# musbenlahrech/reporter

Measured on AMD Instinct MI355X. Metric: GPS points map-matched/sec (node) at 1/2/4/8 MI355X; % of HBM peak, higher is better.
Workload: dtype f32 geometry / f64 Viterbi + times / u64 (dist,time) route keys

## Files before the change

reporter_amd/csrc/engine.hip:

```cpp
#include <hip/hip_runtime.h>
#include <hipcub/hipcub.hpp>

#include <algorithm>
#include <chrono>
#include <cstdlib>
#include <cstring>
#include <functional>
#include <thread>
#include <type_traits>

#include "engine.hpp"
#include "json_points.hpp"

namespace rm {

const char* const kKernelNames[kNumKernels] = {"states", "candidates", "scan", "routes",
                                               "viterbi", "paths", "segments", "report", "locality",
                                               "points"};

namespace {

constexpr uint32_t kEmpty = 0xffffffffu;
constexpr int kWave = 64;
constexpr int kBigH = 4096;
// ... 196 lines not shown
  if (k == 0 && lane < kCtlWords) b.ctl[lane] = 0u;
  const uint32_t o = b.trace_off[k], n = b.trace_off[k + 1] - o;
  const MatchOptions op = b.opts[b.trace_opt[k]];
  const double interp = (double)op.interpolation_distance;
  uint32_t ns = 0, last = 0;
  float llon = 0.f, llat = 0.f;
  double lsin = 0.0, lcos = 0.0;
  float c1lo = 0.f, c1la = 0.f, c2lo = 0.f, c2la = 0.f;
  const uint32_t nl = n ? n - 1u : 0u;
  float nlo = b.lon[o + min((uint32_t)lane, nl)], nla = b.lat[o + min((uint32_t)lane, nl)];
  double ntm = b.time[o + min((uint32_t)lane, nl)];
  bool w_slot = false, w_state = false, w_gc = false;
  uint32_t w_i = 0, w_si = 0;
  double w_gcv = 0.0, w_tm = 0.0;
  for (uint32_t c0 = 0; c0 < n; c0 += 64) {
    const uint32_t i = c0 + lane, m = min(64u, n - c0);
    const bool act = i < n;
    float lo = act ? nlo : 0.f, la = act ? nla : 0.f;
    double tm = act ? ntm : 0.0;
    __asm__ volatile("" : "+v"(lo), "+v"(la), "+v"(tm) : : "memory");
    if (w_slot) { b.slot_trace[o + w_i] = k; b.choice[o + w_i] = -1; b.path_cnt[o + w_i] = 0u; }
    if (w_state) { b.state_orig[o + w_si] = w_i; b.state_time[o + w_si] = w_tm; }
    if (w_gc) b.gc[o + w_si] = w_gcv;
    __asm__ volatile("" : : : "memory");
    nlo = b.lon[o + min(i + 64u, nl)];
    nla = b.lat[o + min(i + 64u, nl)];
    ntm = b.time[o + min(i + 64u, nl)];
    w_slot = act;
    w_i = i;
    float lo1 = __shfl_up(lo, 1, 64), la1 = __shfl_up(la, 1, 64);
    float lo2 = __shfl_up(lo, 2, 64), la2 = __shfl_up(la, 2, 64);
    if (lane == 0) { lo1 = c1lo; la1 = c1la; lo2 = c2lo; la2 = c2la; }
    if (lane == 1) { lo2 = c1lo; la2 = c1la; }
    const double s0 = lat_sin(la), k0 = lat_cos(la);
    double s1 = __shfl_up(s0, 1, 64), k1 = __shfl_up(k0, 1, 64), s2 = __shfl_up(s0, 2, 64), k2 = __shfl_up(k0, 2, 64);
    if (lane <= 1) {
      const float cl = lane == 0 ? c2la : c1la;
      s2 = lat_sin(cl); k2 = lat_cos(cl);
      if (lane == 0) { s1 = lat_sin(c1la); k1 = lat_cos(c1la); }
    }
    const double d1 = gc_trig(lo1, la1, s1, k1, lo, la, s0, k0);
    const double d2 = gc_trig(lo2, la2, s2, k2, lo, la, s0, k0);
    const bool a1 = act && (i == 0 || !(d1 < interp));
    const bool a2 = act && i >= 2 && !(d2 < interp);
    const unsigned long long A = __ballot(a1), B = __ballot(a2);
    unsigned long long st = 0;
    const uint32_t last0 = last;
    double dx = 0.0;
    for (uint32_t q = 0; q < m;) {
      const uint32_t ii = c0 + q;
      if (ii == 0 || last + 1 == ii) {
        const unsigned long long rest = ~(A >> q);
        const uint32_t run = min(rest ? (uint32_t)__builtin_ctzll(rest) : 64u, m - q);
        if (run) {
          st |= (run == 64u ? ~0ull : ((1ull << run) - 1ull)) << q;
          q += run;
          last = c0 + q - 1;
        } else {
          ++q;
        }
        continue;
      }
      if (last + 2 == ii) {
        if ((B >> q) & 1ull) { st |= 1ull << q; last = ii; }
        ++q;
        continue;
      }
      float plo = llon, pla = llat;
      double ps = lsin, pc = lcos;
      if (last >= c0) {
        plo = lane_f(lo, last - c0); pla = lane_f(la, last - c0);
        ps = lane_d(s0, last - c0); pc = lane_d(k0, last - c0);
      }
      const double dv = gc_trig(plo, pla, ps, pc, lo, la, s0, k0);
      const unsigned long long far = __ballot(act && !(dv < interp)) & (~0ull << q);
      if (!far) { q = m; break; }
      const uint32_t nq = (uint32_t)__builtin_ctzll(far);
      st |= 1ull << nq;
      last = c0 + nq;
      if (lane == (int)nq) dx = dv;
      q = nq + 1;
    }
    w_state = ((st >> lane) & 1ull) != 0ull;
    w_tm = tm;
    w_gc = false;
    if (w_state) {
      const unsigned long long below = st & ((1ull << lane) - 1ull);
      const uint32_t si = ns + (uint32_t)__popcll(below);
      w_si = si;
      if (si > 0) {
        const uint32_t prev = below ? c0 + 63u - (uint32_t)__builtin_clzll(below) : last0;
        w_gc = true;
        w_gcv = i - prev == 1u ? d1 : (i - prev == 2u ? d2 : dx);
      }
    }
    ns += (uint32_t)__popcll(st);
    if (last >= c0) {
      llon = lane_f(lo, last - c0); llat = lane_f(la, last - c0);
      lsin = lane_d(s0, last - c0); lcos = lane_d(k0, last - c0);
    }
    c1lo = lane_f(lo, 63); c1la = lane_f(la, 63);
    c2lo = lane_f(lo, 62); c2la = lane_f(la, 62);
  }
  if (w_slot) { b.slot_trace[o + w_i] = k; b.choice[o + w_i] = -1; b.path_cnt[o + w_i] = 0u; }
  if (w_state) { b.state_orig[o + w_si] = w_i; b.state_time[o + w_si] = w_tm; }
  if (w_gc) b.gc[o + w_si] = w_gcv;
  if (lane == 0) b.n_states[k] = ns;
}

struct CandSmem {
  uint32_t road[kCandH];
  unsigned long long best[kCandH];
  uint32_t cell_lo[64], cell_hi[64];
  uint32_t used, ovf, ncell, slot_n;
  uint32_t list[kCandH];
};

__device__ __forceinline__ void project_rel(float ax, float ay, uint32_t acum, float bx, float by, uint32_t bcum,
                                            float& sq, uint32_t& s) {
  const float dx = bx - ax, dy = by - ay;
  const float l2 = dx * dx + dy * dy;
  float t = 0.0f;
  if (l2 > 0.0f) {
    t = -(ax * dx + ay * dy) / l2;
    if (t < 0.0f) t = 0.0f;
    if (t > 1.0f) t = 1.0f;
  }
  const float cx = ax + t * dx, cy = ay + t * dy;
  sq = cx * cx + cy * cy;
  const float along = (float)acum + t * (float)(bcum - acum);
  uint32_t v = (uint32_t)rintf(along);
  if (v < acum) v = acum;
  if (v > bcum) v = bcum;
  s = v;
}
__device__ __forceinline__ void project(float alon, float alat, uint32_t acum, float blon, float blat, uint32_t bcum,
                                        float lon, float lat, float mlon, float mlat, float& sq, uint32_t& s) {
  project_rel((alon - lon) * mlon, (alat - lat) * mlat, acum, (blon - lon) * mlon, (blat - lat) * mlat, bcum, sq, s);
}
#ifndef RM_K1_REJECT
#define RM_K1_REJECT 0
#endif
__device__ __forceinline__ bool outside_pad(float ax, float ay, float bx, float by, float pad) {
  if (!RM_K1_REJECT) return false;
  return (ax > pad && bx > pad) || (ax < -pad && bx < -pad) || (ay > pad && by > pad) || (ay < -pad && by < -pad);
}

__device__ __forceinline__ uint32_t time_ms_dev(uint32_t d_cm, uint32_t dkph) {
  if (d_cm > 11930464u) return time_ms(d_cm, dkph);
  const uint32_t D = dkph ? dkph : 1u;
  return (uint32_t)((double)(d_cm * 360u) / (double)D);
}

__device__ __forceinline__ void desc_from_rec(const uint4& a, const uint4& c, uint32_t road, uint32_t s, int mode,
                                              uint32_t acc, uint4& d0, uint4& d1) {
  uint32_t spf = (a.w != kNone && edge_ok(c.y, acc)) ? mode_speed_dkph(mode, c.y & 0xffffu) : 0u;
  uint32_t spr = (c.x != kNone && edge_ok(c.z, acc)) ? mode_speed_dkph(mode, c.z & 0xffffu) : 0u;
  if (a.w != kNone && edge_ok(c.y, acc) && spf == 0u) spf = 1u;
  if (c.x != kNone && edge_ok(c.z, acc) && spr == 0u) spr = 1u;
  d0 = make_uint4(road, s, a.z, spf | (spr << 16));
  d1 = make_uint4(a.x, a.y, spf ? time_ms_dev(s, spf) : 0xffffffffu, spr ? time_ms_dev(a.z - s, spr) : 0xffffffffu);
}

__device__ __forceinline__ void make_desc(const DevGraph& g, uint32_t road, uint32_t s, int mode, uint4& d0,
                                          uint4& d1) {
  desc_from_rec(g.road_rec[2 * (uint64_t)road], g.road_rec[2 * (uint64_t)road + 1], road, s, mode, mode_access(mode),
                d0, d1);
}

__device__ __forceinline__ void put_cand(const DevGraph& g, const DevBatch& b, uint64_t p, uint32_t rank, uint32_t road,
                                         uint32_t s, float sq, int mode) {
  uint4 d0, d1;
  make_desc(g, road, s, mode, d0, d1);
  const uint64_t at = p * kMaxCand + rank;
  b.cand_desc[2 * at] = d0;
  b.cand_desc[2 * at + 1] = d1;
  b.cand_sq[at] = sq;
}

#define K1_UNIFORM_STOP(c) (__ballot(c) == 0ull)

#ifndef RM_K1_ROWS
#define RM_K1_ROWS 4
#endif
constexpr int kK1Rows = RM_K1_ROWS;
#ifndef RM_K1_BATCH
#define RM_K1_BATCH 4
#endif
constexpr int kK1Batch = RM_K1_BATCH;
#ifndef RM_K1_SLOTS
#define RM_K1_SLOTS 16
#endif
constexpr int kK1Slots = RM_K1_SLOTS;
static_assert(kK1Slots % 4 == 0 && kK1Slots <= kMaxCand, "K1 slots");
#ifndef RM_K1_WPE
#define RM_K1_WPE 1
#endif
__global__ void __launch_bounds__(256) __attribute__((amdgpu_waves_per_eu(RM_K1_WPE))) k_candidates_lane(DevGraph g, DevBatch b) {
  uint64_t p = (uint64_t)blockIdx.x * blockDim.x + threadIdx.x;
  if (b.perm) {
    const uint64_t r = (uint64_t)xcd_block(blockIdx.x, gridDim.x) * blockDim.x + threadIdx.x;
    if (r >= b.P) return;
    p = b.perm[r];
  }
  if (p >= b.P) return;
  const uint32_t k = b.slot_trace[p];
  const uint32_t o = b.trace_off[k];
  const uint32_t s = (uint32_t)(p - o);
  if (s >= b.n_states[k]) return;
  const MatchOptions op = b.opts[b.trace_opt[k]];
  const uint32_t acc = mode_access(op.mode);
  const uint32_t pt = o + b.state_orig[p];
  const float lon = b.lon[pt], lat = b.lat[pt];
  const float r = point_radius(op, b.acc[pt]);
  const float mlon = meters_per_lon(lat);
  const float mlat = (float)kMetersPerDegLat;
  const float r2 = r * r;
  const float pad = r * 1.01f + 0.5f;
  const float qlon = pad / mlon, qlat = pad / mlat;
  const double fx0 = floor(((double)(lon - qlon) - g.lon0) / g.dlon);
  const double fx1 = floor(((double)(lon + qlon) - g.lon0) / g.dlon);
  const double fy0 = floor(((double)(lat - qlat) - g.lat0) / g.dlat);
  const double fy1 = floor(((double)(lat + qlat) - g.lat0) / g.dlat);
  uint32_t rroad[kK1Slots], rs[kK1Slots];
  unsigned long long rbest[kK1Slots];
  uint32_t n = 0;
  bool ovf = false;
  if (!(fx1 < 0 || fy1 < 0 || fx0 > (double)(g.ncx - 1) || fy0 > (double)(g.ncy - 1))) {
    const uint32_t x0 = fx0 < 0 ? 0u : (uint32_t)fx0, y0 = fy0 < 0 ? 0u : (uint32_t)fy0;
    const uint32_t x1 = fx1 > (double)(g.ncx - 1) ? g.ncx - 1 : (uint32_t)fx1;
    const uint32_t y1 = fy1 > (double)(g.ncy - 1) ? g.ncy - 1 : (uint32_t)fy1;
    for (uint32_t w0 = y0; w0 <= y1 && !ovf; w0 += kK1Rows) {
      const uint32_t nrow = min(y1 - w0 + 1u, (uint32_t)kK1Rows);
      uint32_t ra[kK1Rows], re[kK1Rows], base[kK1Rows], end[kK1Rows];
#pragma unroll
      for (int r = 0; r < kK1Rows; ++r) {
        const uint32_t cy = w0 + min((uint32_t)r, nrow - 1u);
        ra[r] = g.cell_off[cy * g.ncx + x0];
        re[r] = g.cell_off[cy * g.ncx + x1 + 1];
      }
      uint32_t tot = 0;
#pragma unroll
      for (int r = 0; r < kK1Rows; ++r) {
        base[r] = ra[r] - tot;
        tot += (uint32_t)r < nrow ? re[r] - ra[r] : 0u;
        end[r] = tot;
      }
      for (uint32_t q0 = 0; q0 < tot && !ovf; q0 += kK1Batch) {
        uint4 r0[kK1Batch], r1[kK1Batch];
#pragma unroll
        for (int y = 0; y < kK1Batch; ++y) {
          const uint32_t q = min(q0 + (uint32_t)y, tot - 1u);
          uint32_t bq = base[0];
#pragma unroll
          for (int r = 1; r < kK1Rows; ++r)
            if (q >= end[r - 1]) bq = base[r];
          const uint64_t it = bq + q;
          r0[y] = g.cell_rec[2 * it];
          r1[y] = g.cell_rec[2 * it + 1];
        }
#pragma unroll
        for (int y = 0; y < kK1Batch; ++y) {
          if (q0 + y >= tot || ovf) break;
          if (!((r1[y].z >> 29) & acc)) continue;
          const float ax = (as_f(r0[y].x) - lon) * mlon, ay = (as_f(r0[y].y) - lat) * mlat;
          const float bx = (as_f(r0[y].z) - lon) * mlon, by = (as_f(r0[y].w) - lat) * mlat;
          if (outside_pad(ax, ay, bx, by, pad)) continue;
          float sq; uint32_t sc;
          project_rel(ax, ay, r1[y].x, bx, by, r1[y].y, sq, sc);
          if (!(sq <= r2)) continue;
          const uint32_t road = r1[y].z & 0x1fffffffu;
          const unsigned long long key = ((unsigned long long)__float_as_uint(sq) << 32) | r1[y].w;
          bool found = false;
#pragma unroll
          for (int x = 0; x < kK1Slots; ++x) {
            if (K1_UNIFORM_STOP(x < (int)n)) break;
            if (x < (int)n && rroad[x] == road) {
              found = true;
              if (key < rbest[x]) { rbest[x] = key; rs[x] = sc; }
            }
          }
          if (found) continue;
          if (n >= (uint32_t)kK1Slots) { ovf = true; break; }
#pragma unroll
          for (int x = 0; x < kK1Slots; ++x) {
            if (K1_UNIFORM_STOP(x <= (int)n)) break;
            if (x == (int)n) { rroad[x] = road; rbest[x] = key; rs[x] = sc; }
          }
          ++n;
        }
      }
    }
  }
  if (ovf) {
    const uint32_t q = atomicAdd(&b.ctl[kCtlK1LaneToWave], 1u);
    b.rl_cand[q] = (uint32_t)p;
    return;
  }
  const uint32_t cacc = mode_access(op.mode);
#pragma unroll
  for (int x0 = 0; x0 < kK1Slots; x0 += 4) {
    if (K1_UNIFORM_STOP(x0 < (int)n)) break;
    if (x0 >= (int)n) break;
    uint4 ra[4], rc[4];
#pragma unroll
    for (int y = 0; y < 4; ++y) {
      const uint64_t road = rroad[min(x0 + y, (int)n - 1)];
      ra[y] = g.road_rec[2 * road];
      rc[y] = g.road_rec[2 * road + 1];
    }
#pragma unroll
    for (int y = 0; y < 4; ++y) {
      const int x = x0 + y;
      if (x >= (int)n) break;
      const uint32_t sqb = (uint32_t)(rbest[x] >> 32);
      const unsigned long long kx = ((unsigned long long)sqb << 32) | rroad[x];
      uint32_t rank = 0;
#pragma unroll
      for (int z = 0; z < kK1Slots; ++z) {
        if (K1_UNIFORM_STOP(z < (int)n)) break;
        if (z >= (int)n) continue;
        rank += ((((rbest[z] >> 32) << 32) | rroad[z]) < kx) ? 1u : 0u;
      }
      uint4 d0, d1;
      desc_from_rec(ra[y], rc[y], rroad[x], rs[x], op.mode, cacc, d0, d1);
      const uint64_t at = p * kMaxCand + rank;
      b.cand_desc[2 * at] = d0;
      b.cand_desc[2 * at + 1] = d1;
      b.cand_sq[at] = __uint_as_float(sqb);
    }
  }
  b.cand_n[p] = (uint8_t)n;
}

__device__ void cand_wave_one(const DevGraph& g, const DevBatch& b, CandSmem& sm, uint64_t p) {
  const int lane = threadIdx.x;
  const uint32_t k = b.slot_trace[p];
  const uint32_t o = b.trace_off[k];
  const MatchOptions op = b.opts[b.trace_opt[k]];
  const uint32_t acc = mode_access(op.mode);
  const uint32_t pt = o + b.state_orig[p];
  const float lon = b.lon[pt], lat = b.lat[pt];
  const float r = point_radius(op, b.acc[pt]);
  const float mlon = meters_per_lon(lat);
  const float mlat = (float)kMetersPerDegLat;
  const float r2 = r * r;
  const float pad = r * 1.01f + 0.5f;
  const float qlon = pad / mlon, qlat = pad / mlat;
  const double fx0 = floor(((double)(lon - qlon) - g.lon0) / g.dlon);
  const double fx1 = floor(((double)(lon + qlon) - g.lon0) / g.dlon);
  const double fy0 = floor(((double)(lat - qlat) - g.lat0) / g.dlat);
  const double fy1 = floor(((double)(lat + qlat) - g.lat0) / g.dlat);
  for (int h = lane; h < kCandH; h += kWave) { sm.road[h] = kEmpty; sm.best[h] = ~0ull; }
  if (lane == 0) { sm.used = 0; sm.ovf = 0; }
  __syncthreads();
  uint32_t n_found = 0;
  if (!(fx1 < 0 || fy1 < 0 || fx0 > (double)(g.ncx - 1) || fy0 > (double)(g.ncy - 1))) {
    const uint32_t x0 = fx0 < 0 ? 0u : (uint32_t)fx0, y0 = fy0 < 0 ? 0u : (uint32_t)fy0;
    const uint32_t x1 = fx1 > (double)(g.ncx - 1) ? g.ncx - 1 : (uint32_t)fx1;
    const uint32_t y1 = fy1 > (double)(g.ncy - 1) ? g.ncy - 1 : (uint32_t)fy1;
    const uint32_t nx = x1 - x0 + 1, ncell = nx * (y1 - y0 + 1);
    for (uint32_t c0 = 0; c0 < ncell; c0 += kWave) {
      const uint32_t c = c0 + lane;
      uint32_t lo = 0, cnt = 0;
      if (c < ncell) {
        const uint32_t cell = (y0 + c / nx) * g.ncx + (x0 + c % nx);
        lo = g.cell_off[cell];
        cnt = g.cell_off[cell + 1] - lo;
      }
      uint32_t incl = cnt;
#pragma unroll
      for (int d = 1; d < kWave; d <<= 1) {
        const uint32_t u = __shfl_up(incl, d, kWave);
        if (lane >= d) incl += u;
      }
      const uint32_t tot = (uint32_t)__shfl((int)incl, kWave - 1, kWave);
      sm.cell_lo[lane] = lo;
      sm.cell_hi[lane] = incl;
      __syncthreads();
      {
        for (uint32_t f = lane; f < tot; f += kWave) {
          uint32_t a = 0, e = kWave - 1;
          while (a < e) {
            const uint32_t mid = (a + e) >> 1;
            if (sm.cell_hi[mid] > f) e = mid;
            else a = mid + 1;
          }
          const uint32_t it = sm.cell_lo[a] + (f - (a ? sm.cell_hi[a - 1] : 0u));
          const uint4 r0 = g.cell_rec[2 * (uint64_t)it], r1 = g.cell_rec[2 * (uint64_t)it + 1];
          if (!((r1.z >> 29) & acc)) continue;
          const float ax = (as_f(r0.x) - lon) * mlon, ay = (as_f(r0.y) - lat) * mlat;
          const float bx = (as_f(r0.z) - lon) * mlon, by = (as_f(r0.w) - lat) * mlat;
          if (outside_pad(ax, ay, bx, by, pad)) continue;
          float sq; uint32_t sc;
          project_rel(ax, ay, r1.x, bx, by, r1.y, sq, sc);
          if (!(sq <= r2)) continue;
          const uint32_t road = r1.z & 0x1fffffffu, v = r1.w;
          uint32_t h = (road * 2654435761u) & (kCandH - 1);
          for (int probe = 0; probe < kCandH; ++probe) {
            uint32_t cur = sm.road[h];
            if (cur == kEmpty) {
              cur = atomicCAS(&sm.road[h], kEmpty, road);
              if (cur == kEmpty) {
                const uint32_t u = atomicAdd(&sm.used, 1u);
                sm.list[u] = h;
                cur = road;
              }
            }
            if (cur == road) {
              atomicMin(&sm.best[h], ((unsigned long long)__float_as_uint(sq) << 32) | v);
              break;
            }
            h = (h + 1) & (kCandH - 1);
          }
        }
      }
      __syncthreads();
    }
    n_found = sm.used;
  }
  if (n_found > kCandH * 3 / 4) {
    if (lane == 0) trace_fail(b, p, kErrCandOverflow);
    n_found = 0;
  }
  for (uint32_t q = lane; q < n_found; q += kWave) {
    const uint32_t h = sm.list[q];
    const uint32_t road = sm.road[h];
    const unsigned long long bst = sm.best[h];
    const uint32_t sqb = (uint32_t)(bst >> 32);
    uint32_t rank = 0;
    for (uint32_t q2 = 0; q2 < n_found; ++q2) {
      const uint32_t h2 = sm.list[q2];
      const uint32_t sqb2 = (uint32_t)(sm.best[h2] >> 32), road2 = sm.road[h2];
      rank += (sqb2 < sqb || (sqb2 == sqb && road2 < road)) ? 1u : 0u;
    }
    if (rank < (uint32_t)kMaxCand) {
      const uint32_t v = (uint32_t)bst;
      const uint4 A = g.verts[v], B = g.verts[v + 1];
      float sq; uint32_t sc;
      project(as_f(A.x), as_f(A.y), A.z, as_f(B.x), as_f(B.y), B.z, lon, lat, mlon, mlat, sq, sc);
      put_cand(g, b, p, rank, road, sc, sq, op.mode);
    }
  }
  if (lane == 0) b.cand_n[p] = (uint8_t)min(n_found, (uint32_t)kMaxCand);
}

__global__ void __launch_bounds__(64) k_candidates_wave(DevGraph g, DevBatch b, int all) {
  __shared__ CandSmem sm;
  const uint32_t n_items = all ? (uint32_t)b.P : min(b.ctl[kCtlK1LaneToWave], (uint32_t)b.P);
  for (uint32_t item = blockIdx.x; item < n_items; item += gridDim.x) {
    const uint32_t p = all ? item : b.rl_cand[item];
    if (all) {
      const uint32_t k = b.slot_trace[p];
      if (p - b.trace_off[k] >= b.n_states[k]) continue;
    }
    cand_wave_one(g, b, sm, p);
    __syncthreads();
  }
}

__device__ __forceinline__ void block_sum2_u64(unsigned long long a, unsigned long long c, unsigned long long* part) {
  __shared__ unsigned long long sa[4], sc[4];
#pragma unroll
  for (int d = 32; d > 0; d >>= 1) {
    a += __shfl_down(a, d, 64);
    c += __shfl_down(c, d, 64);
  }
  if ((threadIdx.x & 63) == 0) { sa[threadIdx.x >> 6] = a; sc[threadIdx.x >> 6] = c; }
  __syncthreads();
  if (threadIdx.x == 0)
    reinterpret_cast<ulonglong2*>(part)[blockIdx.x] =
        make_ulonglong2(sa[0] + sa[1] + sa[2] + sa[3], sc[0] + sc[1] + sc[2] + sc[3]);
}

__device__ __forceinline__ void block_excl_scan2(unsigned long long a, unsigned long long c, unsigned long long& ea,
                                                 unsigned long long& ec, unsigned long long* sa, unsigned long long* sc,
                                                 int nwaves) {
  const int lane = threadIdx.x & 63, wv = threadIdx.x >> 6;
  unsigned long long ia = a, ic = c;
#pragma unroll
  for (int d = 1; d < 64; d <<= 1) {
    const unsigned long long ta = __shfl_up(ia, d, 64), tc = __shfl_up(ic, d, 64);
    if (lane >= d) { ia += ta; ic += tc; }
  }
  if (lane == 63) { sa[wv] = ia; sc[wv] = ic; }
// ... 302 lines not shown
    for (uint32_t q = 0; q < c; ++q)
      if (o + q < b.seg_cap) rec_slot[o + q] = (uint32_t)(i + j);
    o += c;
  }
  if (blockIdx.x == gridDim.x - 1 && threadIdx.x == 255) tot[2] = base + mine;
}

__global__ void __launch_bounds__(64) k_gather_recs(uint32_t T, const uint32_t* base, const uint32_t* cnt,
                                                    const uint32_t* off, const unsigned long long* src, uint32_t words,
                                                    unsigned long long* dst) {
  for (uint32_t k = blockIdx.x; k < T; k += gridDim.x) {
    const uint64_t n = (uint64_t)cnt[k] * words;
    const unsigned long long* s = src + (uint64_t)base[k] * words;
    unsigned long long* d = dst + (uint64_t)off[k] * words;
    for (uint64_t q = threadIdx.x; q < n; q += 64) d[q] = s[q];
  }
}

__global__ void __launch_bounds__(1024) k_seg_offsets_small(DevBatch b, uint32_t* off) {
  __shared__ unsigned long long sa[16], sc[16];
  const uint32_t T = b.T;
  const bool off_gate = small_abort(b);
  const uint32_t per = (T + 1023u) / 1024u;
  const uint32_t k0 = min(threadIdx.x * per, T), k1 = min(k0 + per, T);
  unsigned long long a = 0;
  for (uint32_t k = k0; k < k1; ++k) a += off_gate ? 0u : b.seg_cnt[k];
  unsigned long long ea, ec;
  block_excl_scan2(a, 0ull, ea, ec, sa, sc, 16);
  for (uint32_t k = k0; k < k1; ++k) {
    off[k] = (uint32_t)ea;
    if (off_gate) b.seg_cnt[k] = 0u;
    else ea += b.seg_cnt[k];
  }
  if (threadIdx.x == 1023) off[T] = (uint32_t)ea;
}

__device__ __forceinline__ uint32_t d_spf(const uint4& d0) { return d0.w & 0xffffu; }
__device__ __forceinline__ uint32_t d_spr(const uint4& d0) { return d0.w >> 16; }

__device__ __forceinline__ unsigned long long route_key_vals(const uint4& a0, const uint4& b0, const uint4& b1,
                                                             unsigned long long lab0, unsigned long long lab1,
                                                             int* combo) {
  const uint32_t sa = a0.y, rb = b0.x, sb = b0.y, L = b0.z, spf = d_spf(b0), spr = d_spr(b0);
  unsigned long long best = kKeyInf;
  int bc = -1;
  if (a0.x == rb) {
    const bool fw = sb > sa || (sb == sa && spf);
    const uint32_t sp = fw ? spf : spr, d = fw ? sb - sa : sa - sb;
    if (sp) { best = make_key(d, time_ms_dev(d, sp)); bc = fw ? 0 : 1; }
  }
  if (spf && lab0 != kKeyInf) { const unsigned long long k = lab0 + make_key(sb, b1.z); if (k < best) { best = k; bc = 2; } }
  if (spr && lab1 != kKeyInf) { const unsigned long long k = lab1 + make_key(L - sb, b1.w); if (k < best) { best = k; bc = 3; } }
  if (combo) *combo = bc;
  return best;
}

template <class Label>
__device__ __forceinline__ unsigned long long route_key(const Label& label, const uint4& a0, const uint4& b0,
                                                        const uint4& b1, int* combo) {
  const unsigned long long lab0 = d_spf(b0) ? label(b1.x) : kKeyInf;
  const unsigned long long lab1 = d_spr(b0) ? label(b1.y) : kKeyInf;
  return route_key_vals(a0, b0, b1, lab0, lab1, combo);
}

__device__ __forceinline__ void exit_keys(const uint4& a0, uint32_t bound, unsigned long long& rk1,
                                          unsigned long long& rk0) {
  const uint32_t s = a0.y, L = a0.z, spf = d_spf(a0), spr = d_spr(a0);
  rk1 = (spf && L - s <= bound) ? make_key(L - s, time_ms_dev(L - s, spf)) : kKeyInf;
  rk0 = (spr && s <= bound) ? make_key(s, time_ms_dev(s, spr)) : kKeyInf;
}

template <int H, bool PATH>
struct SearchSmem {
  using FIdx = typename std::conditional<(H >= 65536), uint32_t, uint16_t>::type;
  uint32_t key[H];
  unsigned long long lab[H];
  FIdx fa[H], fb[H];
  uint32_t inq[(H + 31) / 32];
  uint32_t pred[PATH ? H : 1];
  uint32_t nf, nn, used, ovf;
};

__device__ __forceinline__ bool inq_set(uint32_t* inq, uint32_t slot) {
  const uint32_t bit = 1u << (slot & 31);
  return (atomicOr(&inq[slot >> 5], bit) & bit) == 0u;
}
__device__ __forceinline__ void inq_clear(uint32_t* inq, uint32_t slot) { atomicAnd(&inq[slot >> 5], ~(1u << (slot & 31))); }

template <int H, bool PATH>
__device__ __forceinline__ int h_insert(SearchSmem<H, PATH>& sm, uint32_t key) {
  uint32_t h = (key * 2654435761u) & (H - 1);
  for (int probe = 0; probe < H; ++probe) {
    uint32_t cur = sm.key[h];
    if (cur == key) return (int)h;
    if (cur == kEmpty) {
      cur = atomicCAS(&sm.key[h], kEmpty, key);
      if (cur == kEmpty) {
        if (atomicAdd(&sm.used, 1u) >= (uint32_t)(H * 3 / 4)) sm.ovf = 1u;
        return (int)h;
      }
      if (cur == key) return (int)h;
    }
    h = (h + 1) & (H - 1);
  }
  sm.ovf = 1u;
  return -1;
}

template <int H, bool PATH>
__device__ __forceinline__ int h_find(const SearchSmem<H, PATH>& sm, uint32_t key) {
  uint32_t h = (key * 2654435761u) & (H - 1);
  for (int probe = 0; probe < H; ++probe) {
    const uint32_t cur = sm.key[h];
    if (cur == key) return (int)h;
    if (cur == kEmpty) return -1;
    h = (h + 1) & (H - 1);
  }
  return -1;
}

template <int H, bool PATH>
__device__ __forceinline__ unsigned long long h_label(const SearchSmem<H, PATH>& sm, uint32_t key) {
  const int h = h_find(sm, key);
  return h < 0 ? kKeyInf : sm.lab[h];
}

__device__ __forceinline__ uint32_t wave_append(uint32_t* counter) {
  const unsigned long long m = __ballot(1);
  const int lane = (int)(threadIdx.x & (kWave - 1));
  const int leader = __builtin_ctzll(m);
  uint32_t base = 0;
  if (lane == leader) base = atomicAdd(counter, (uint32_t)__popcll(m));
  base = (uint32_t)__shfl((int)base, leader, kWave);
  return base + (uint32_t)__popcll(m & ((1ull << lane) - 1ull));
}

template <int H, bool PATH>
struct HashLabel {
  const SearchSmem<H, PATH>& sm;
  uint32_t srcbits;
  __device__ unsigned long long operator()(uint32_t node) const { return h_label(sm, srcbits | node); }
};
template <int H, bool PATH>
struct HashPathLabel {
  const SearchSmem<H, PATH>& sm;
  __device__ unsigned long long operator()(uint32_t node, uint32_t, uint32_t) const { return h_label(sm, node); }
};

struct SearchTargets {
  const uint4* tg;
  uint32_t n;
  uint32_t delta;
};

__device__ __forceinline__ void wave_sync() {
  __builtin_amdgcn_fence(__ATOMIC_RELEASE, "wavefront");
  __builtin_amdgcn_wave_barrier();
  __builtin_amdgcn_fence(__ATOMIC_ACQUIRE, "wavefront");
}

template <int W>
__device__ __forceinline__ void grp_sync() {
  if constexpr (W == kWave) __syncthreads();
  else wave_sync();
}
template <int W>
__device__ __forceinline__ int grp_lane() { return (int)(threadIdx.x & (W - 1)); }
template <int W>
__device__ __forceinline__ int grp_base() { return (int)(threadIdx.x & (kWave - 1) & ~(W - 1)); }
template <int W>
__device__ __forceinline__ unsigned long long grp_ballot(bool x) {
  const unsigned long long m = __ballot(x);
  if constexpr (W == kWave) return m;
  else return (m >> grp_base<W>()) & ((1ull << W) - 1ull);
}
template <int W>
__device__ __forceinline__ uint32_t grp_append(uint32_t* counter) {
  if constexpr (W == kWave) {
    return wave_append(counter);
  } else {
    const unsigned long long m = grp_ballot<W>(true);
    const int j = grp_lane<W>();
    const int leader = __builtin_ctzll(m);
    uint32_t base = 0;
    if (j == leader) base = atomicAdd(counter, (uint32_t)__popcll(m));
    base = (uint32_t)__shfl((int)base, grp_base<W>() + leader, kWave);
    return base + (uint32_t)__popcll(m & ((1ull << j) - 1ull));
  }
}
template <int W>
__device__ __forceinline__ unsigned long long grp_min_u64(unsigned long long v) {
#pragma unroll
  for (int d = W / 2; d >= 1; d >>= 1) {
    const unsigned long long o = ((unsigned long long)(uint32_t)__shfl_xor((int)(v >> 32), d, W) << 32) |
                                 (uint32_t)__shfl_xor((int)(uint32_t)v, d, W);
    v = o < v ? o : v;
  }
  return v;
}

template <int H, bool PATH, int W = kWave>
__device__ void bounded_search(SearchSmem<H, PATH>& sm, const DevGraph& g, int mode, uint32_t bound,
                               const uint4* src, uint32_t n_src, uint32_t root = 0,
                               SearchTargets tgt = SearchTargets{nullptr, 0u, kNone}) {
  using FIdx = typename SearchSmem<H, PATH>::FIdx;
  constexpr FIdx kDeferred = (FIdx)~(FIdx)0;
  static_assert((uint64_t)H <= (uint64_t)kDeferred, "frontier index needs a spare value");
  static_assert(W == kWave || W == 16, "64 or 16 lanes per search");
  const int lane = grp_lane<W>();
  const uint32_t acc = mode_access(mode);
  for (int h = lane; h < H; h += W) {
    sm.key[h] = kEmpty; sm.lab[h] = kKeyInf;
    if ((h & 31) == 0) sm.inq[h >> 5] = 0u;
    if (PATH) sm.pred[h] = kNone;
  }
  if (lane == 0) { sm.nf = 0; sm.nn = 0; sm.used = 0; sm.ovf = 0; }
  const bool has_tg = tgt.tg != nullptr && tgt.n != 0u;
  uint4 t0 = make_uint4(0u, 0u, 0u, 0u), t1 = t0;
  if (has_tg && (uint32_t)lane < tgt.n) { t0 = tgt.tg[2 * lane]; t1 = tgt.tg[2 * lane + 1]; }
  const bool use_min = has_tg || tgt.delta != kNone;
  grp_sync<W>();
  if (!src) {
    if (lane == 0) {
      const int slot = h_insert(sm, root);
      sm.lab[slot] = 0ull;
      sm.inq[slot >> 5] |= 1u << (slot & 31);
      sm.fa[sm.nf++] = (FIdx)slot;
    }
  } else if ((uint32_t)lane < 2u * n_src) {
    const uint32_t i = lane >> 1;
    const uint4 a0 = src[2 * i], a1 = src[2 * i + 1];
    unsigned long long rk1, rk0;
    exit_keys(a0, bound, rk1, rk0);
    const unsigned long long kk = (lane & 1) ? rk0 : rk1;
    if (kk != kKeyInf) {
      const uint32_t node = (lane & 1) ? a1.x : a1.y;
      const int slot = h_insert(sm, (i << 28) | node);
      if (slot >= 0) {
        const unsigned long long old = atomicMin(&sm.lab[slot], kk);
        if (kk < old && inq_set(sm.inq, slot)) sm.fa[grp_append<W>(&sm.nf)] = (FIdx)slot;
      }
    }
  }
  grp_sync<W>();
  const uint4 sa0 = src ? src[0] : make_uint4(0u, 0u, 0u, 0u);
  for (int round = 0;; ++round) {
    const uint32_t nf = sm.nf;
    if (nf == 0 || sm.ovf) break;
    if (round > 4 * H) { if (lane == 0) sm.ovf = 2u; break; }
    FIdx* cur = (round & 1) ? sm.fb : sm.fa;
    FIdx* nxt = (round & 1) ? sm.fa : sm.fb;
    unsigned long long thr = kKeyInf;
    if (use_min) {
      unsigned long long fm = kKeyInf;
      for (uint32_t q = lane; q < nf; q += W) {
        const unsigned long long l = sm.lab[cur[q]];
        fm = l < fm ? l : fm;
      }
      fm = grp_min_u64<W>(fm);
      if (has_tg) {
        bool done = true;
        if ((uint32_t)lane < tgt.n) done = route_key(HashLabel<H, PATH>{sm, 0u}, sa0, t0, t1, nullptr) < fm;
        if (grp_ballot<W>(!done) == 0ull) break;
      }
      if (tgt.delta != kNone) thr = fm + ((unsigned long long)tgt.delta << 32);
    }
    if (thr == kKeyInf) {
      for (uint32_t q = lane; q < nf; q += W) inq_clear(sm.inq, cur[q]);
    } else {
      for (uint32_t q = lane; q < nf; q += W) {
        const FIdx slot = cur[q];
        if (sm.lab[slot] > thr) {
          nxt[grp_append<W>(&sm.nn)] = slot;
          cur[q] = kDeferred;
        } else {
          inq_clear(sm.inq, slot);
        }
      }
    }
    grp_sync<W>();
    for (uint32_t q = lane; q < nf; q += W) {
      const FIdx fs = cur[q];
      if (fs == kDeferred) continue;
      const int slot = fs;
      const uint32_t kk = sm.key[slot];
      const uint32_t node = kk & 0x0fffffffu, srcbits = kk & 0xf0000000u;
      const unsigned long long lab = sm.lab[slot];
      const uint32_t e0 = g.node_off[node], e1 = g.node_off[node + 1];
      for (uint32_t e = e0; e < e1; ++e) {
        const uint4 rec = g.edges[e];
        if (!edge_ok(rec.z, acc)) continue;
        const unsigned long long nk = lab + edge_key(rec, mode);
        if (key_dist(nk) > bound) continue;
        const int t = h_insert(sm, srcbits | rec.x);
        if (t < 0) continue;
        const unsigned long long old = atomicMin(&sm.lab[t], nk);
        if (nk < old && inq_set(sm.inq, (uint32_t)t)) nxt[grp_append<W>(&sm.nn)] = (FIdx)t;
      }
    }
    grp_sync<W>();
    if (lane == 0) { sm.nf = sm.nn; sm.nn = 0; }
    grp_sync<W>();
  }
  grp_sync<W>();
}

#ifndef RM_LANE_CAP
#define RM_LANE_CAP 7
#endif
constexpr int kLaneCap = RM_LANE_CAP;
#ifndef RM_LANE_WPE
#define RM_LANE_WPE 4
// ... 4628 lines not shown
```

Measured before the change: 2.078 billion.

## Compact K1 candidate epilogue across wave via LDS staging and nontemporal stores

```diff
diff --git a/reporter_amd/csrc/engine.hip b/reporter_amd/csrc/engine.hip
--- a/reporter_amd/csrc/engine.hip
+++ b/reporter_amd/csrc/engine.hip
@@ -372,6 +372,24 @@
   return (uint32_t)((double)(d_cm * 360u) / (double)D);
 }
 
+#ifndef RM_K1_EPILOGUE
+#define RM_K1_EPILOGUE 1
+#endif
+
+__device__ __noinline__ uint32_t time_ms_far(uint32_t d_cm, uint32_t dkph) { return time_ms(d_cm, dkph); }
+__device__ __forceinline__ uint32_t time_ms_wave(uint32_t d_cm, uint32_t dkph) {
+#if RM_K1_EPILOGUE == 1
+  const uint32_t D = dkph ? dkph : 1u;
+  uint32_t t = (uint32_t)((double)(d_cm * 360u) / (double)D);
+  if (__ballot(d_cm > 11930464u) != 0ull) {
+    if (d_cm > 11930464u) t = time_ms_far(d_cm, dkph);
+  }
+  return t;
+#else
+  return time_ms_dev(d_cm, dkph);
+#endif
+}
+
 __device__ __forceinline__ void desc_from_rec(const uint4& a, const uint4& c, uint32_t road, uint32_t s, int mode,
                                               uint32_t acc, uint4& d0, uint4& d1) {
   uint32_t spf = (a.w != kNone && edge_ok(c.y, acc)) ? mode_speed_dkph(mode, c.y & 0xffffu) : 0u;
@@ -379,7 +397,8 @@
   if (a.w != kNone && edge_ok(c.y, acc) && spf == 0u) spf = 1u;
   if (c.x != kNone && edge_ok(c.z, acc) && spr == 0u) spr = 1u;
   d0 = make_uint4(road, s, a.z, spf | (spr << 16));
-  d1 = make_uint4(a.x, a.y, spf ? time_ms_dev(s, spf) : 0xffffffffu, spr ? time_ms_dev(a.z - s, spr) : 0xffffffffu);
+  const uint32_t tf = time_ms_wave(s, spf), tr = time_ms_wave(a.z - s, spr);
+  d1 = make_uint4(a.x, a.y, spf ? tf : 0xffffffffu, spr ? tr : 0xffffffffu);
 }
 
 __device__ __forceinline__ void make_desc(const DevGraph& g, uint32_t road, uint32_t s, int mode, uint4& d0,
@@ -399,6 +418,12 @@
 }
 
 #define K1_UNIFORM_STOP(c) (__ballot(c) == 0ull)
+
+__device__ __forceinline__ void wave_sync() {
+  __builtin_amdgcn_fence(__ATOMIC_RELEASE, "wavefront");
+  __builtin_amdgcn_wave_barrier();
+  __builtin_amdgcn_fence(__ATOMIC_ACQUIRE, "wavefront");
+}
 
 #ifndef RM_K1_ROWS
 #define RM_K1_ROWS 4
@@ -416,14 +441,27 @@
 #ifndef RM_K1_WPE
 #define RM_K1_WPE 1
 #endif
-__global__ void __launch_bounds__(256) __attribute__((amdgpu_waves_per_eu(RM_K1_WPE))) k_candidates_lane(DevGraph g, DevBatch b) {
-  uint64_t p = (uint64_t)blockIdx.x * blockDim.x + threadIdx.x;
-  if (b.perm) {
-    const uint64_t r = (uint64_t)xcd_block(blockIdx.x, gridDim.x) * blockDim.x + threadIdx.x;
-    if (r >= b.P) return;
-    p = b.perm[r];
-  }
-  if (p >= b.P) return;
+#ifndef RM_K1_STAGE
+#define RM_K1_STAGE 384
+#endif
+constexpr int kK1Stage = RM_K1_STAGE;
+static_assert(kK1Stage >= 1, "K1 stage");
+#ifndef RM_K1_NT
+#define RM_K1_NT 1
+#endif
+#ifndef RM_K1_ONESCAN
+#define RM_K1_ONESCAN 0
+#endif
+
+__device__ __forceinline__ uint64_t k1_slot(const DevBatch& b) {
+  if (!b.perm) return (uint64_t)blockIdx.x * blockDim.x + threadIdx.x;
+  const uint64_t r = (uint64_t)xcd_block(blockIdx.x, gridDim.x) * blockDim.x + threadIdx.x;
+  return r < b.P ? (uint64_t)b.perm[r] : b.P;
+}
+
+__device__ __forceinline__ void k1_gather(const DevGraph& g, const DevBatch& b, uint64_t p, uint32_t (&rroad)[kK1Slots],
+                                          uint32_t (&rs)[kK1Slots], unsigned long long (&rbest)[kK1Slots], uint32_t& n,
+                                          bool& ovf) {
   const uint32_t k = b.slot_trace[p];
   const uint32_t o = b.trace_off[k];
   const uint32_t s = (uint32_t)(p - o);
@@ -442,10 +480,6 @@
   const double fx1 = floor(((double)(lon + qlon) - g.lon0) / g.dlon);
   const double fy0 = floor(((double)(lat - qlat) - g.lat0) / g.dlat);
   const double fy1 = floor(((double)(lat + qlat) - g.lat0) / g.dlat);
-  uint32_t rroad[kK1Slots], rs[kK1Slots];
-  unsigned long long rbest[kK1Slots];
-  uint32_t n = 0;
-  bool ovf = false;
   if (!(fx1 < 0 || fy1 < 0 || fx0 > (double)(g.ncx - 1) || fy0 > (double)(g.ncy - 1))) {
     const uint32_t x0 = fx0 < 0 ? 0u : (uint32_t)fx0, y0 = fy0 < 0 ? 0u : (uint32_t)fy0;
     const uint32_t x1 = fx1 > (double)(g.ncx - 1) ? g.ncx - 1 : (uint32_t)fx1;
@@ -492,6 +526,23 @@
           const uint32_t road = r1[y].z & 0x1fffffffu;
           const unsigned long long key = ((unsigned long long)__float_as_uint(sq) << 32) | r1[y].w;
           bool found = false;
+#if RM_K1_ONESCAN
+#pragma unroll
+          for (int x = 0; x < kK1Slots; ++x) {
+            if (K1_UNIFORM_STOP(x <= (int)n)) break;
+            if (x < (int)n) {
+              if (rroad[x] == road) {
+                found = true;
+                if (key < rbest[x]) { rbest[x] = key; rs[x] = sc; }
+              }
+            } else if (x == (int)n && !found) {
+              rroad[x] = road; rbest[x] = key; rs[x] = sc;
+            }
+          }
+          if (found) continue;
+          if (n >= (uint32_t)kK1Slots) { ovf = true; break; }
+          ++n;
+#else
 #pragma unroll
           for (int x = 0; x < kK1Slots; ++x) {
             if (K1_UNIFORM_STOP(x < (int)n)) break;
@@ -508,16 +559,101 @@
             if (x == (int)n) { rroad[x] = road; rbest[x] = key; rs[x] = sc; }
           }
           ++n;
+#endif
         }
       }
     }
   }
+}
+
+struct K1Stage {
+  uint4 rec[4][kK1Stage];
+  uint64_t p[4][kWave];
+};
+
+__global__ void __launch_bounds__(256) __attribute__((amdgpu_waves_per_eu(RM_K1_WPE))) k_candidates_lane(DevGraph g, DevBatch b) {
+  uint32_t rroad[kK1Slots], rs[kK1Slots];
+  unsigned long long rbest[kK1Slots];
+  uint32_t n = 0;
+  bool ovf = false;
+  {
+    const uint64_t p = k1_slot(b);
+    if (p < b.P) k1_gather(g, b, p, rroad, rs, rbest, n, ovf);
+  }
+  const uint64_t p = k1_slot(b);
+  const bool live = p < b.P && (uint32_t)(p - b.trace_off[b.slot_trace[p]]) < b.n_states[b.slot_trace[p]];
+  const int mode = live ? b.opts[b.trace_opt[b.slot_trace[p]]].mode : 0;
   if (ovf) {
     const uint32_t q = atomicAdd(&b.ctl[kCtlK1LaneToWave], 1u);
     b.rl_cand[q] = (uint32_t)p;
-    return;
-  }
-  const uint32_t cacc = mode_access(op.mode);
+    n = 0;
+  }
+#if RM_K1_EPILOGUE == 1
+  uint32_t rank[kK1Slots];
+#pragma unroll
+  for (int x = 0; x < kK1Slots; ++x) rank[x] = 0;
+#pragma unroll
+  for (int z = 1; z < kK1Slots; ++z) {
+    if (K1_UNIFORM_STOP(z < (int)n)) break;
+    if (z < (int)n) {
+      const unsigned long long kz = ((rbest[z] >> 32) << 32) | rroad[z];
+#pragma unroll
+      for (int x = 0; x < z; ++x) {
+        const bool c = kz < (((rbest[x] >> 32) << 32) | rroad[x]);
+        rank[x] += c ? 1u : 0u;
+        rank[z] += c ? 0u : 1u;
+      }
+    }
+  }
+  __shared__ K1Stage sm;
+  const int lane = threadIdx.x & (kWave - 1), wv = threadIdx.x >> 6;
+  uint32_t incl = n;
+#pragma unroll
+  for (int d = 1; d < kWave; d <<= 1) {
+    const uint32_t u = __shfl_up(incl, d, kWave);
+    if (lane >= d) incl += u;
+  }
+  const uint32_t tot = (uint32_t)__shfl((int)incl, kWave - 1, kWave);
+  const uint32_t first = incl - n;
+  sm.p[wv][lane] = p;
+  const uint32_t tag = (uint32_t)lane | ((uint32_t)mode << 16);
+  for (uint32_t f0 = 0; f0 < tot; f0 += (uint32_t)kK1Stage) {
+#pragma unroll
+    for (int x = 0; x < kK1Slots; ++x) {
+      if (K1_UNIFORM_STOP(x < (int)n)) break;
+      const uint32_t f = first + (uint32_t)x - f0;
+      if (x < (int)n && f < (uint32_t)kK1Stage)
+        sm.rec[wv][f] = make_uint4(rroad[x], rs[x], (uint32_t)(rbest[x] >> 32), tag | (rank[x] << 8));
+    }
+    wave_sync();
+    const uint32_t cnt = min(tot - f0, (uint32_t)kK1Stage);
+#pragma unroll 1
+    for (uint32_t i = (uint32_t)lane; i < cnt; i += kWave) {
+      const uint4 c = sm.rec[wv][i];
+      const uint4 ra = g.road_rec[2 * (uint64_t)c.x], rc = g.road_rec[2 * (uint64_t)c.x + 1];
+      const int cm = (int)(c.w >> 16);
+      uint4 d0, d1;
+      desc_from_rec(ra, rc, c.x, c.y, cm, mode_access(cm), d0, d1);
+      const uint64_t at = sm.p[wv][c.w & 63u] * kMaxCand + ((c.w >> 8) & 15u);
+#if RM_K1_NT
+      typedef uint32_t K1V4 __attribute__((ext_vector_type(4)));
+      __builtin_nontemporal_store((K1V4){d0.x, d0.y, d0.z, d0.w}, (K1V4*)&b.cand_desc[2 * at]);
+      __builtin_nontemporal_store((K1V4){d1.x, d1.y, d1.z, d1.w}, (K1V4*)&b.cand_desc[2 * at + 1]);
+      __builtin_nontemporal_store(c.z, (uint32_t*)&b.cand_sq[at]);
+#else
+      b.cand_desc[2 * at] = d0;
+      b.cand_desc[2 * at + 1] = d1;
+      b.cand_sq[at] = __uint_as_float(c.z);
+#endif
+    }
+    wave_sync();
+  }
+  if (live && !ovf) b.cand_n[p] = (uint8_t)n;
+#elif RM_K1_EPILOGUE == 2
+  if (live && !ovf) b.cand_n[p] = (uint8_t)n;
+#else
+  if (!live || ovf) return;
+  const uint32_t cacc = mode_access(mode);
 #pragma unroll
   for (int x0 = 0; x0 < kK1Slots; x0 += 4) {
     if (K1_UNIFORM_STOP(x0 < (int)n)) break;
@@ -543,7 +679,7 @@
         rank += ((((rbest[z] >> 32) << 32) | rroad[z]) < kx) ? 1u : 0u;
       }
       uint4 d0, d1;
-      desc_from_rec(ra[y], rc[y], rroad[x], rs[x], op.mode, cacc, d0, d1);
+      desc_from_rec(ra[y], rc[y], rroad[x], rs[x], mode, cacc, d0, d1);
       const uint64_t at = p * kMaxCand + rank;
       b.cand_desc[2 * at] = d0;
       b.cand_desc[2 * at + 1] = d1;
@@ -551,6 +687,7 @@
     }
   }
   b.cand_n[p] = (uint8_t)n;
+#endif
 }
 
 __device__ void cand_wave_one(const DevGraph& g, const DevBatch& b, CandSmem& sm, uint64_t p) {
@@ -1159,12 +1296,6 @@
   uint32_t n;
   uint32_t delta;
 };
-
-__device__ __forceinline__ void wave_sync() {
-  __builtin_amdgcn_fence(__ATOMIC_RELEASE, "wavefront");
-  __builtin_amdgcn_wave_barrier();
-  __builtin_amdgcn_fence(__ATOMIC_ACQUIRE, "wavefront");
-}
 
 template <int W>
 __device__ __forceinline__ void grp_sync() {
```

Result: faster. 2.146 billion (median of 6 runs) (+3.3%).
